# MaxInGaussian/SCFGP

Hardware: AMD Instinct MI355X
Metric: NLML+grad evals/sec (higher is better)
Workload: dtype f32

## Files before the change

### scfgp_amd/csrc/fmap.hip

```cpp
#include "kernels.h"
#include "tile_engine.h"

#include <algorithm>

#define SMEM_DECL extern __shared__ __attribute__((aligned(16))) char smem_raw[]
#ifndef SCFGP_FMAP_WGM
#define SCFGP_FMAP_WGM 4
#endif
#ifndef SCFGP_FMAP_MIN_WGS
#define SCFGP_FMAP_MIN_WGS 6144
#endif
#ifndef SCFGP_FMAP_REG
#define SCFGP_FMAP_REG 1
#endif
#ifndef SCFGP_FMAP_REG_MIN_WGS
#define SCFGP_FMAP_REG_MIN_WGS 16384
#endif
typedef TileCfg<double, 128, 64, 16, SCFGP_FMAP_WGM, 2, 16, true> FmapCfg;

template <typename T>
__global__ __launch_bounds__(FmapCfg::THREADS) void featuremap_kernel(
    const double* __restrict__ Xt, const double* __restrict__ Fall, const Scal* __restrict__ sc,
    T* __restrict__ Phi, int Dp, int Jp, int Kp, int J, int64_t N, int njt, int ncs) {
    typedef FmapCfg Cfg;
    SMEM_DECL;
    double* smem = reinterpret_cast<double*>(smem_raw);
    const int cs = blockIdx.x % ncs;
    const int64_t rb = blockIdx.x / ncs;
    const int per = (njt + ncs - 1) / ncs, jt0 = cs * per, nseg = (jt0 + per <= njt ? per : njt - jt0);
    if (nseg <= 0) return;
    const int nkt = Dp / Cfg::BK;
    TrLoader<double, double, Cfg::BM, Cfg::BK, Cfg::LDA, Cfg::THREADS, false, Cfg::SWZA> la(Xt + rb * Cfg::BM * Dp, Dp, threadIdx.x);
    NatLoader<double, double, Cfg::BN, Cfg::BK, Cfg::LDB, Cfg::THREADS, false, false> lb(Fall + jt0 * Cfg::BN, Jp, threadIdx.x);
    typename Cfg::MTr::acc_t acc[Cfg::TM][Cfg::TN];
    acc_zero<Cfg>(acc);
    const double s = sc->s;
    const T s_hi = (T)s, s_lo = (T)(s - (double)s_hi);
    AccCoord<Cfg> co;
    tile_mainloop_segments<Cfg>(la, lb, nkt, nseg, -(int64_t)Dp, (int64_t)Cfg::BN - (int64_t)Dp * Jp, acc, smem,
        [&](int seg, typename Cfg::MTr::acc_t (&a)[Cfg::TM][Cfg::TN]) {
            T vs[Cfg::TM][Cfg::TN][Cfg::MTr::NACC], vc[Cfg::TM][Cfg::TN][Cfg::MTr::NACC];
#pragma unroll
            for (int tm = 0; tm < Cfg::TM; ++tm)
#pragma unroll
                for (int tn = 0; tn < Cfg::TN; ++tn)
#pragma unroll
                    for (int r = 0; r < Cfg::MTr::NACC; ++r) {
                        T sn, cs_;
                        fast_sincos(a[tm][tn][r], sn, cs_);
                        vc[tm][tn][r] = fma(cs_, s_hi, cs_ * s_lo);
                        vs[tm][tn][r] = fma(sn, s_hi, sn * s_lo);
                    }
#pragma unroll
            for (int tm = 0; tm < Cfg::TM; ++tm)
#pragma unroll
                for (int r = 0; r < Cfg::MTr::NACC; ++r) {
                    const int64_t n = rb * Cfg::BM + co.row(tm, r);
                    T* __restrict__ prow = Phi + n * Kp;
#pragma unroll
                    for (int tn = 0; tn < Cfg::TN; ++tn) {
                        const int j = (jt0 + seg) * Cfg::BN + co.col(tn);
                        if (j < J) {
                            prow[j] = n < N ? vc[tm][tn][r] : (T)0;
                            prow[J + j] = n < N ? vs[tm][tn][r] : (T)0;
                        }
                    }
                }
        });
}

template <typename T, int NK>
__global__ __launch_bounds__(256) void featuremap_reg_kernel(
    const double* __restrict__ A, int lda, const double* __restrict__ Fall, const Scal* __restrict__ sc,
    T* __restrict__ Phi, int Jp, int Kp, int J, int64_t N, int nct, int ncs) {
    typedef MT<double, 16> M;
    typedef T tv2 __attribute__((ext_vector_type(2)));
    const int lane = threadIdx.x & 63, wave = threadIdx.x >> 6, q = lane >> 4, i = lane & 15;
    const int cs = blockIdx.x % ncs;
    const int64_t rb = blockIdx.x / ncs;
    const int per = (nct + ncs - 1) / ncs, ct0 = cs * per, nseg = ct0 + per <= nct ? per : nct - ct0;
    if (nseg <= 0) return;
    const int64_t row0 = rb * 128 + wave * 32;
    double a[2][NK];
#pragma unroll
    for (int tm = 0; tm < 2; ++tm)
#pragma unroll
        for (int ks = 0; ks < NK; ++ks) a[tm][ks] = A[(row0 + tm * 16 + i) * lda + ks * 4 + q];
    const double* bp = Fall + (int64_t)q * Jp + ct0 * 32 + 2 * i;
    v2d b[NK];
#pragma unroll
    for (int ks = 0; ks < NK; ++ks) b[ks] = *reinterpret_cast<const v2d*>(bp + (int64_t)ks * 4 * Jp);
    const double s = sc->s;
    const T s_hi = (T)s, s_lo = (T)(s - (double)s_hi);
    const bool vec = (J & 1) == 0;
    for (int seg = 0; seg < nseg; ++seg) {
        v4d acc[2][2];
#pragma unroll
        for (int tm = 0; tm < 2; ++tm)
#pragma unroll
            for (int tn = 0; tn < 2; ++tn) acc[tm][tn] = v4d{0, 0, 0, 0};
#pragma unroll
        for (int ks = 0; ks < NK; ++ks)
#pragma unroll
            for (int tm = 0; tm < 2; ++tm)
#pragma unroll
                for (int tn = 0; tn < 2; ++tn) M::mfma(acc[tm][tn], a[tm][ks], b[ks][tn]);
        bp += 32;
        if (seg + 1 < nseg) {
#pragma unroll
            for (int ks = 0; ks < NK; ++ks) b[ks] = *reinterpret_cast<const v2d*>(bp + (int64_t)ks * 4 * Jp);
        }
        const int c = (ct0 + seg) * 32 + 2 * i;
        T vs[2][4][2], vc[2][4][2];
#pragma unroll
        for (int tm = 0; tm < 2; ++tm)
#pragma unroll
            for (int r = 0; r < 4; ++r)
#pragma unroll
                for (int tn = 0; tn < 2; ++tn) {
                    T sn, cs_;
                    fast_sincos(acc[tm][tn][r], sn, cs_);
                    vc[tm][r][tn] = fma(cs_, s_hi, cs_ * s_lo);
                    vs[tm][r][tn] = fma(sn, s_hi, sn * s_lo);
                }
#pragma unroll
        for (int tm = 0; tm < 2; ++tm)
#pragma unroll
            for (int r = 0; r < 4; ++r) {
                const int64_t n = row0 + tm * 16 + M::crow(lane, r);
                T* __restrict__ prow = Phi + n * Kp;
                const bool live = n < N;
                const T c0 = live ? vc[tm][r][0] : (T)0, c1 = live ? vc[tm][r][1] : (T)0;
                const T s0 = live ? vs[tm][r][0] : (T)0, s1 = live ? vs[tm][r][1] : (T)0;
                if (vec) {
                    if (c < J) {
                        *reinterpret_cast<tv2*>(prow + c) = tv2{c0, c1};
                        *reinterpret_cast<tv2*>(prow + J + c) = tv2{s0, s1};
                    }
                } else {
                    if (c < J) { prow[c] = c0; prow[J + c] = s0; }
                    if (c + 1 < J) { prow[c + 1] = c1; prow[J + c + 1] = s1; }
                }
            }
    }
}

__global__ __launch_bounds__(FmapCfg::THREADS) void project_kernel(
    const double* __restrict__ Xt, const double* __restrict__ Lall, double* __restrict__ Tt, int Dp, int Sp, int Spp, int njt) {
    typedef FmapCfg Cfg;
    SMEM_DECL;
    double* smem = reinterpret_cast<double*>(smem_raw);
    const int jt = blockIdx.x % njt;
    const int64_t rb = blockIdx.x / njt;
    TrLoader<double, double, Cfg::BM, Cfg::BK, Cfg::LDA, Cfg::THREADS, false, Cfg::SWZA> la(Xt + rb * Cfg::BM * Dp, Dp, threadIdx.x);
    NatLoader<double, double, Cfg::BN, Cfg::BK, Cfg::LDB, Cfg::THREADS, false, false> lb(Lall + jt * Cfg::BN, Spp, threadIdx.x);
    typename Cfg::MTr::acc_t acc[Cfg::TM][Cfg::TN];
    acc_zero<Cfg>(acc);
    tile_mainloop<Cfg>(la, lb, Dp / Cfg::BK, acc, smem);
    AccCoord<Cfg> co;
#pragma unroll
    for (int tm = 0; tm < Cfg::TM; ++tm)
#pragma unroll
        for (int tn = 0; tn < Cfg::TN; ++tn) {
            const int j = jt * Cfg::BN + co.col(tn);
            if (j >= Sp) continue;
#pragma unroll
            for (int r = 0; r < Cfg::MTr::NACC; ++r) Tt[(rb * Cfg::BM + co.row(tm, r)) * Sp + j] = acc[tm][tn][r];
        }
}

template <typename T>
void FmapKernels<T>::featuremap(const Geom& g, const double* Xt, const Projection& pr, const Scal* sc, T* Phi, hipStream_t st) {
    const int njt = g.Jp / FmapCfg::BN;
    const int64_t nrb = g.Np / FmapCfg::BM;
    int ncs = (int)std::min<int64_t>(njt, std::max<int64_t>(1, (SCFGP_FMAP_MIN_WGS + nrb - 1) / nrb));
    const auto launch = [&](auto kernel, const double* A, const double* Bm, int Kd) {
        allow_big_lds(kernel, FmapCfg::LDS_BYTES);
        hipLaunchKernelGGL(kernel, dim3((unsigned)(ncs * nrb)), dim3(FmapCfg::THREADS), FmapCfg::LDS_BYTES, st,
                           A, Bm, sc, Phi, Kd, g.Jp, g.Kp, g.J, g.N, njt, ncs);
    };
    const double *A = Xt, *Bm = pr.Fall; int Kd = g.Dp;
    if (g.lowrank) {
        const int Spp = (int)round_up(g.Sp, FmapCfg::BN), njs = Spp / FmapCfg::BN;
        allow_big_lds(project_kernel, FmapCfg::LDS_BYTES);
        hipLaunchKernelGGL(project_kernel, dim3((unsigned)(njs * nrb)), dim3(FmapCfg::THREADS), FmapCfg::LDS_BYTES, st,
                           Xt, pr.Lall, pr.Tt, g.Dp, g.Sp, Spp, njs);
        A = pr.Tt; Bm = pr.Rall; Kd = g.Sp;
    }
    const int live = (g.lowrank ? g.S : g.D) + 1, nk = (live + 3) / 4;
    if (SCFGP_FMAP_REG && nk <= 9) {
        const int nct = g.Jp / 32;
        const int rcs = (int)std::min<int64_t>(nct, std::max<int64_t>(1, (SCFGP_FMAP_REG_MIN_WGS + nrb - 1) / nrb));
        const auto reg = [&](auto kernel) {
            hipLaunchKernelGGL(kernel, dim3((unsigned)(rcs * nrb)), dim3(256), 0, st, A, Kd, Bm, sc, Phi, g.Jp, g.Kp, g.J, g.N, nct, rcs);
        };
        if (nk <= 3 && Kd >= 12) { reg(featuremap_reg_kernel<T, 3>); return; }
        if (nk <= 4 && Kd >= 16) { reg(featuremap_reg_kernel<T, 4>); return; }
        if (nk <= 5 && Kd >= 20) { reg(featuremap_reg_kernel<T, 5>); return; }
        if (nk <= 8 && Kd >= 32) { reg(featuremap_reg_kernel<T, 8>); return; }
        if (Kd >= 36) { reg(featuremap_reg_kernel<T, 9>); return; }
    }
    launch(featuremap_kernel<T>, A, Bm, Kd);
}

template <typename T>
__global__ void convert_kernel(const double* __restrict__ src, T* __restrict__ dst, int K, int Kp) {
    const int64_t n = (int64_t)Kp * Kp;
    for (int64_t i = (int64_t)blockIdx.x * blockDim.x + threadIdx.x; i < n; i += (int64_t)gridDim.x * blockDim.x) {
        const int r = (int)(i / Kp), c = (int)(i % Kp);
        dst[i] = (r < K && c < K) ? (T)src[i] : (T)0;
    }
}
template <typename T>
__global__ void convert_t_kernel(const double* __restrict__ src, T* __restrict__ dst, int K, int Kp) {
    const int64_t n = (int64_t)Kp * Kp;
    for (int64_t i = (int64_t)blockIdx.x * blockDim.x + threadIdx.x; i < n; i += (int64_t)gridDim.x * blockDim.x) {
        const int k = (int)(i / Kp), j = (int)(i % Kp);
        dst[i] = (k < K && j < K) ? (T)src[(int64_t)j * Kp + k] : (T)0;
    }
}
template <typename T>
void FmapKernels<T>::convert_transposed(const double* src, T* dst, int K, int Kp, hipStream_t st) {
    hipLaunchKernelGGL(convert_t_kernel<T>, dim3(2048), dim3(256), 0, st, src, dst, K, Kp);
}
template <typename T>
void FmapKernels<T>::convert(const double* src, T* dst, int K, int Kp, hipStream_t st) {
    hipLaunchKernelGGL(convert_kernel<T>, dim3(2048), dim3(256), 0, st, src, dst, K, Kp);
}
template struct FmapKernels<double>;
template struct FmapKernels<float>;
__device__ __forceinline__ double scale_x(double x, int mode, const double* __restrict__ sp, int D, int d) {
    if (mode == 0) return x;
    const double mn = sp[d], mx = sp[D + d], lm = sp[2 * D + d], mu = sp[3 * D + d], sd = sp[4 * D + d];
    if (mode == 1) return (x - mn) / (mx - mn);
    if (mode == 2) return (x - mu) / sd;
    if (mode == 3) return 0.5 * erfc(-((x - mu) / sd) * 0.70710678118654752440);
    const double t = (x - mn) / (mx - mn);
    const double bc = ((t < 0 ? -1.0 : (t > 0 ? 1.0 : 0.0)) * pow(fabs(t), lm) - 1.0) / lm;
    const double z = (bc - mu) / sd;
    return mode == 4 ? z : 0.5 * erfc(-z * 0.70710678118654752440);
}
__device__ __forceinline__ double scale_x_deriv(double x, int mode, const double* __restrict__ sp, int D, int d) {
    if (mode == 0) return 1.0;
    const double mn = sp[d], mx = sp[D + d], lm = sp[2 * D + d], mu = sp[3 * D + d], sd = sp[4 * D + d];
    const double inv_sqrt_2pi = 0.39894228040143267794;
// ... 48 lines not shown
```

### scfgp_amd/csrc/kernels.h

```cpp
#pragma once
#include "common.h"

struct Geom {
    int D, S, M, J, K, P;
    int Dp;
    int Jp;
    int Sp;
    int lowrank;
    int Kp;
    int tile;
    int gfull;
    int gstrip;
    int64_t N;
    int64_t Np;
};

struct RowSplits {
    int nsplit;
    int groups;
    int units;
    int taper;
    int gran;
    int64_t nrb;
    __host__ __device__ int per_group() const { return units + taper; }
    __host__ __device__ void range(int s, int64_t& r0, int64_t& r1) const {
        const int pg = per_group(), grp = s / pg, i = s % pg;
        const int64_t g0 = nrb * grp / groups, g1 = nrb * (grp + 1) / groups, len = g1 - g0;
        const int64_t den = (int64_t)1 << taper;
        const int k = i - (units - 1);
        int64_t e0, e1;
        if (taper == 0 || k < 0) { e0 = den * i; e1 = e0 + den; }
        else {
            const int64_t base = den * (units - 1);
            e0 = base + den - (den >> k);
            e1 = k == taper ? base + den : base + den - (den >> (k + 1));
        }
        r0 = (g0 + len * e0 / (den * units)) * gran;
        r1 = (g0 + len * e1 / (den * units)) * gran;
    }
};
RowSplits gram_row_splits(int jobs_per_split, int64_t Np, bool f32, int nsplit_override, int taper);

struct Projection { const double* Fall; const double* Lall; const double* Rall; double* Tt; };

template <typename T>
struct FmapKernels {
    static void featuremap(const Geom& g, const double* Xt, const Projection& pr, const Scal* sc, T* Phi, hipStream_t st);
    static void convert(const double* src, T* dst, int K, int Kp, hipStream_t st);
    static void convert_transposed(const double* src, T* dst, int K, int Kp, hipStream_t st);
};

template <typename T>
struct GramKernels {
    static void gram(const Geom& g, const T* Phi, const double* w, const double* side, const RowSplits& rs, int64_t chunk,
                     double* slabs, double* sidepart, int* qhead, float* ws2, hipStream_t st);
    static int gram_jobs(const Geom& g);
    static void xtz(const Geom& g, const double* Xt, const T* Phi, const T* Phibar, int nsplit, int64_t chunk, double* slabs,
                    hipStream_t st);
    static void zbar_inplace(const Geom& g, const T* Phi, T* Phibar, hipStream_t st);
    static void rsel(const Geom& g, const double* params, T* out, hipStream_t st);
    static void tn_plain(const double* A, int Dp, const T* Bm, int64_t ldb, int J, int64_t Np, int nsplit, int64_t chunk, double* slabs,
                         hipStream_t st);
};

struct F16Operands { const unsigned* Phi16; const char* B16; const float* scale; unsigned* V16; const float* vbound; };

template <typename T>
struct ApplyKernels {
    static void apply_v(const Geom& g, const T* Phi, const T* Bm, T* V, double* vpart, const double* alpha, double* mupart,
                        hipStream_t st, int dma = 0, const F16Operands* f16 = nullptr);
    static void apply_predict(const Geom& g, const T* Phi, const T* LiT, double* vpart, const double* alpha, double* mupart,
                              hipStream_t st);
    static void apply_c(const Geom& g, const T* Phi, const T* LiT, const T* Li, T* C, double* vpart, const double* alpha,
                        const double* beta, double* mupart, hipStream_t st, int dma = 0);
    static void apply_vc(const Geom& g, const T* C, const T* Li, const T* LiT, T* V, hipStream_t st, int dma = 0);
    static void apply_phibar(const Geom& g, const T* Phi, const T* Abar, T* V, const double* p, const double* q,
                             const double* y, const double* alpha, const double* ut, hipStream_t st, int dma = 0, const F16Operands* f16 = nullptr);
    static void apply_plain(const Geom& g, const T* A, const T* Bm, T* Out, int Kc, int ncols, hipStream_t st);
    static void rowstats(const Geom& g, const double* mupart, const double* vpart, const double* y,
                         const Scal* sc, double* p, double* q, double* partial, int nblocks, hipStream_t st);
    static void rowpredict(const Geom& g, const double* mupart, const double* vpart, const Scal* sc, double* mu, double* sd,
                           hipStream_t st);
    static void rowresidual(const Geom& g, const double* mupart, const double* y, double* r, hipStream_t st);
};

struct F16x3Kernels {
    static void split_operand(const Geom& g, const double* M, char* B16, float* scale, double* part, const Scal* sc, hipStream_t st);
    template <int EPI, int BN>
    static int apply(const Geom& g, int njt, int col0, int slot0, const float* Phi, const F16Operands& f, float* V,
                     double* vpart, const double* p, const double* q, const double* y, const double* alpha, const double* ut, double* mu,
                     hipStream_t st, int64_t rb0, int64_t nrb);
    static bool apply_runs(const Geom& g);
    static constexpr size_t F16_PAD = 1024;
    static int side_blocks(const Geom& g);
    static void split_phi(const Geom& g, const float* Phi, const double* y, const Scal* sc, unsigned* Phi16, double* sidepart, float* tmp,
                          hipStream_t st);
// ... 126 lines not shown
```

### scfgp_amd/csrc/scfgp_api.hip

```cpp
#include "../../include/scfgp_hip.h"
#include "kernels.h"

#include <dlfcn.h>
#if __has_include(<rccl/rccl.h>)
#include <rccl/rccl.h>
#else
extern "C" {
typedef struct ncclComm* ncclComm_t;
typedef struct { char internal[128]; } ncclUniqueId;
typedef enum { ncclSuccess = 0 } ncclResult_t;
typedef enum { ncclFloat64 = 8 } ncclDataType_t;
typedef enum { ncclSum = 0 } ncclRedOp_t;
ncclResult_t ncclGetUniqueId(ncclUniqueId*);
ncclResult_t ncclCommInitRank(ncclComm_t*, int, ncclUniqueId, int);
ncclResult_t ncclAllReduce(const void*, void*, size_t, ncclDataType_t, ncclRedOp_t, ncclComm_t, hipStream_t);
ncclResult_t ncclCommDestroy(ncclComm_t);
const char* ncclGetErrorString(ncclResult_t);
}
#endif

#include <algorithm>
#include <cmath>
#include <cstdlib>
#include <cstring>
// ... 20 lines not shown
#ifndef SCFGP_ERR_PER_COND
#define SCFGP_ERR_PER_COND 3.0e-7
#endif
static void derive_geom(Geom& g, int D, int S, int M);

thread_local bool g_scfgp_capturing = false;

struct Roctx {
    int (*push)(const char*) = nullptr; int (*pop)() = nullptr;
    Roctx() {
        void* h = dlopen("librocprofiler-sdk-roctx.so", RTLD_LAZY | RTLD_LOCAL);
        if (!h) h = dlopen("libroctx64.so", RTLD_LAZY | RTLD_LOCAL);
        if (!h) return;
        push = (int (*)(const char*))dlsym(h, "roctxRangePushA");
        pop = (int (*)())dlsym(h, "roctxRangePop");
        if (!push || !pop) { push = nullptr; pop = nullptr; }
    }
};
static Roctx& roctx() { static Roctx r; return r; }

struct Rccl {
    void* h = nullptr;
    decltype(&ncclGetUniqueId) get_id = nullptr; decltype(&ncclCommInitRank) init_rank = nullptr;
    decltype(&ncclAllReduce) all_reduce = nullptr; decltype(&ncclCommDestroy) destroy = nullptr;
    decltype(&ncclGetErrorString) err_string = nullptr;
    bool resolved = false;
    bool bind(void* from) {
        get_id = (decltype(get_id))dlsym(from, "ncclGetUniqueId"); init_rank = (decltype(init_rank))dlsym(from, "ncclCommInitRank");
        all_reduce = (decltype(all_reduce))dlsym(from, "ncclAllReduce"); destroy = (decltype(destroy))dlsym(from, "ncclCommDestroy");
        err_string = (decltype(err_string))dlsym(from, "ncclGetErrorString");
        return get_id && init_rank && all_reduce && destroy && err_string;
    }
    Rccl() {
        if (dlsym(RTLD_DEFAULT, "ncclAllReduce") && bind(RTLD_DEFAULT)) { resolved = true; return; }
        const char* names[] = {"librccl.so", "librccl.so.1", "/opt/rocm/lib/librccl.so.1"};
        for (const char* n : names) if (!h) h = dlopen(n, RTLD_NOW | RTLD_NOLOAD | RTLD_LOCAL);
        for (const char* n : names) if (!h) h = dlopen(n, RTLD_NOW | RTLD_LOCAL);
        if (!h) return;
        if (bind(h)) resolved = true;
        else { dlclose(h); h = nullptr; }
    }
    bool ok() const { return resolved; }
};
static Rccl& rccl() { static Rccl r; return r; }

struct ProfRec { std::string name; hipEvent_t e0, e1; };

struct scfgp_ctx {
    Geom g{};
    int dtype = 0, device = 0;
    hipStream_t st = nullptr; bool own_stream = false;
    hipStream_t copy_st = nullptr; hipEvent_t ev_factor = nullptr;
    int lowrank_bwd = -1; int Spp = 0, Sq = 0; bool last_lrb = false;
    bool want_lrb() const {
        const bool fits = g.lowrank && g.Jp + (int)round_up(g.S, 64) <= g.Kp;
        return fits && (lowrank_bwd == 1 || (lowrank_bwd < 0 && g.Dp >= 4 * g.Sp));
    }
    double* x3_scalars() { return d_x3 + (int64_t)Dpp * g.Jp; }
    double* xs1() { return d_xp1 + n_pk + g.Kp; }
    double* xs2() { return d_xp2 + n_pk + g.Kp; }
    bool unsettled = false; int test_deny_level = 0, test_fail_stage = 0;
    int cap() const { return esc_denied > 0 ? esc_denied - 1 : 2; }
    double* x3_xu() { return d_x3 + (int64_t)Dpp * g.Jp + 8; }
    hipEvent_t ev_fence = nullptr;
    ncclComm_t comm = nullptr; int comm_ranks = 0, comm_rank = 0;
    double* h_pin = nullptr;
    int64_t Ncap = 0, Nglobal = 0, Nglobal_full = 0;
    bool have_params = false, have_data = false;
    int stage = 0, last_want_grad = 0;
    std::vector<double> h_params;
    double *d_params = nullptr, *d_F = nullptr, *d_Fall = nullptr, *d_Lall = nullptr, *d_Rall = nullptr; Scal* d_sc = nullptr;
    double *d_Tt = nullptr, *p_Tt = nullptr;
    double *d_Xraw = nullptr, *d_yraw = nullptr; int64_t Nstore = 0, store_cap = 0; bool work_full = false;
    int64_t* d_idx = nullptr; int64_t idx_cap = 0;
    double *d_Xt = nullptr, *d_y = nullptr, *d_p = nullptr, *d_q = nullptr, *d_mu = nullptr, *d_vpart = nullptr;
    void *d_Phi = nullptr, *d_V = nullptr;
    bool split16 = false; unsigned* d_Phi16 = nullptr; char* d_B16 = nullptr; float* d_f16scale = nullptr;
    unsigned* d_V16g = nullptr; unsigned* d_qV16g = nullptr; double* d_f16side = nullptr; float* d_f16tmp = nullptr;
    int f16gram = 1;
    bool f16_on() const { return split16 && dma() == 2; }
    int64_t f16_chunk() const {
        const int64_t top = gram_chunk > 0 ? 2 * gram_chunk : 8192, fill = g.Np * F16x3Kernels::gram_tiles(g) / 512 / 512 * 512;
        return std::max<int64_t>(std::min(top, fill), 1024);
    }
    bool f16_gram() const { return f16_on() && f16gram && !last_cform; }
    F16Operands f16ops() const { return F16Operands{d_Phi16, d_B16, d_f16scale, nullptr, d_f16tmp + 5}; }
    double *d_xp1 = nullptr, *d_xp2 = nullptr; int64_t n_xp = 0, n_pk = 0;
    double *d_x1 = nullptr, *d_x2 = nullptr, *d_x3 = nullptr; int64_t n_x1 = 0, n_x2 = 0, n_x3 = 0; int Dpp = 0;
    double *d_Li = nullptr, *d_B = nullptr, *d_T1 = nullptr, *d_T2 = nullptr, *d_Abar = nullptr;
    void *d_BT = nullptr, *d_AbarT = nullptr;
    int apply_dma = -1;
    double *d_vecs = nullptr;
    double *d_scalars = nullptr, *d_yy = nullptr; int* d_flag = nullptr;
    float* d_ws2 = nullptr;
    double *d_slabs = nullptr; size_t slabs_bytes = 0;
    double *d_partial = nullptr; int64_t n_partial = 0;
    double *d_work = nullptr, *d_grad = nullptr;
    int xs_mode = 0; double* d_xscale = nullptr;
    int ys_mode = 0; double* d_yscale = nullptr;
    double *p_Xt = nullptr, *p_vpart = nullptr, *p_mupart = nullptr; void *p_Phi = nullptr;
    void *p_FT = nullptr, *p_C = nullptr, *p_V = nullptr, *p_Li = nullptr;
    double *u_Li = nullptr, *u_S = nullptr, *u_Lm = nullptr, *u_Mi = nullptr, *u_Si = nullptr, *u_vec = nullptr, *u_acc = nullptr, *u_part = nullptr;
    double *u_y = nullptr, *u_r = nullptr, *u_slabs = nullptr; size_t u_slabs_bytes = 0;
    void* u_LiT = nullptr; float* u_ws2 = nullptr; int* u_flag = nullptr;
    double *l_y = nullptr, *l_r = nullptr, *l_rec = nullptr, *l_out = nullptr, *l_acc = nullptr; unsigned long long* l_bad = nullptr;
    int opt_algo = -1; OptHyper opt_h{}; double *d_opt = nullptr, *d_tctr = nullptr, *d_hist = nullptr; int hist_cap = 0;
// ... 287 lines not shown
        dfree(c->d_Xraw); dfree(c->d_yraw); c->store_cap = 0;
        if (int rc = dmalloc(c, &c->d_Xraw, sizeof(double) * N * c->g.D)) return rc;
        if (int rc = dmalloc(c, &c->d_yraw, sizeof(double) * N)) return rc;
        c->store_cap = N;
    }
    c->Nstore = N; c->Nglobal_full = n_global > 0 ? n_global : N;
    HIPCHK(c, hipMemcpyAsync(c->d_Xraw, X, sizeof(double) * N * c->g.D, hipMemcpyHostToDevice, c->st));
    HIPCHK(c, hipMemcpyAsync(c->d_yraw, y, sizeof(double) * N, hipMemcpyHostToDevice, c->st));
    if (int rc = load_working_set(c, nullptr, N, n_global)) return rc;
    HIPCHK(c, hipStreamSynchronize(c->st));
    return SCFGP_OK;
}

static void unpack_exchange(scfgp_ctx* c, const double* xp, double* x) {
    const Geom& g = c->g;
    unpack_tri_tiles(xp, g.Kp / g.tile, g.tile, x, g.Kp, c->st);
    hipMemcpyAsync(x + (int64_t)g.Kp * g.Kp, xp + c->n_pk, sizeof(double) * (g.Kp + 8), hipMemcpyDeviceToDevice, c->st);
}

template <typename T> struct Impl {
    typedef SweepKernels<T> SK;
    static void gram_to(scfgp_ctx* c, const T* Mx, const double* w, const double* side, double* out, const char* name) {
        const Geom& g = c->g;
        const int nts = g.Kp / g.tile, ntiles = nts * (nts + 1) / 2;
        if constexpr (sizeof(T) == 4) {
            if (c->f16_gram()) {
                const int nch = F16x3Kernels::gram_chunks(g, c->f16_chunk());
                { ProfScope ps(c, w ? "split_v" : "split_phi");
                  if (w) F16x3Kernels::split_v(g, (const float*)Mx, w, side, F16x3Kernels::apply_runs(g) ? nullptr : c->d_V16g, c->d_qV16g,
                                               c->d_f16side, c->d_f16tmp, c->st);
                  else F16x3Kernels::split_phi(g, (const float*)Mx, side, c->d_sc, c->d_Phi16, c->d_f16side, c->d_f16tmp, c->st); }
                { ProfScope ps(c, name);
                  F16x3Kernels::gram(g, w ? c->d_V16g : c->d_Phi16, w ? c->d_qV16g : c->d_Phi16, c->d_f16tmp + 4, c->f16_chunk(), c->d_slabs, c->st); }
                { ProfScope ps(c, "reduce_tiles"); reduce_tri_tiles(c->d_slabs, nch, nts, g.tile, out, c->st);
                  reduce_side(c->d_f16side, F16x3Kernels::side_blocks(g), g.Kp, g.gfull * g.tile + g.gstrip * 64, out + c->n_pk, c->st); }
                return;
            }
        }
        const int gs = c->splits.nsplit;
        double* sidepart = c->d_slabs + (size_t)gs * ntiles * g.tile * g.tile;
        { ProfScope ps(c, name);
          SK::gram(g, Mx, w, side, c->splits, c->dtype == SCFGP_F32 ? c->gram_chunk : 0, c->d_slabs, sidepart, c->d_flag + 8, c->d_ws2, c->st); }
        { ProfScope ps(c, "reduce_tiles"); reduce_tri_tiles(c->d_slabs, gs, nts, g.tile, out, c->st);
          reduce_side(sidepart, gs, g.Kp, g.gfull * g.tile + g.gstrip * 64, out + c->n_pk, c->st); }
    }
    static int pass1(scfgp_ctx* c) {
        const Geom& g = c->g;
        if (!c->in_train) HIPCHK(c, hipMemsetAsync(c->d_flag, 0, sizeof(int) * 4, c->st));
        const bool use64 = sizeof(T) == 4 && c->use64();
        c->last_cform = c->want_cform();
        if ((use64 && c->phi64_cap < g.Np) || (c->last_cform && c->c_cap < g.Np)) {
            c->err = "pass1: auxiliary row buffer missing"; return SCFGP_EARG;
        }
        const Projection proj{c->d_Fall, c->d_Lall, c->d_Rall, c->d_Tt};
        if constexpr (sizeof(T) == 4) {
            if (use64) {
                typedef SweepKernels<double> SK64;
                const int nts = g.Kp / g.tile, ntiles = nts * (nts + 1) / 2, gs = c->splits64.nsplit;
                double* sidepart = c->d_slabs + (size_t)gs * ntiles * g.tile * g.tile;
                { ProfScope ps(c, "featuremap64"); SK64::featuremap(g, c->d_Xt, proj, c->d_sc, (double*)c->d_Phi64, c->st); }
                { ProfScope ps(c, "gram64");
                  SK64::gram(g, (const double*)c->d_Phi64, nullptr, c->d_y, c->splits64, 0, c->d_slabs, sidepart, c->d_flag + 8, nullptr, c->st); }
                { ProfScope ps(c, "reduce_tiles"); reduce_tri_tiles(c->d_slabs, gs, nts, g.tile, c->d_xp1, c->st);
                  reduce_side(sidepart, gs, g.Kp, g.gfull * g.tile + g.gstrip * 64, c->d_xp1 + c->n_pk, c->st); }
            }
        }
        { ProfScope ps(c, "featuremap"); SK::featuremap(g, c->d_Xt, proj, c->d_sc, (T*)c->d_Phi, c->st); }
        if constexpr (sizeof(T) == 4) {
            if (c->f16_on() && (use64 || !c->f16_gram())) {
                ProfScope ps(c, "split_phi");
                F16x3Kernels::split_phi(g, (const float*)c->d_Phi, c->d_y, c->d_sc, c->d_Phi16, c->d_f16side, c->d_f16tmp, c->st);
            }
        }
        if (!use64) gram_to(c, (const T*)c->d_Phi, nullptr, c->d_y, c->d_xp1, "gram");
        c->last_used64 = use64 || sizeof(T) == 8; c->last_level = sizeof(T) == 8 ? 0 : c->level();
        HIPCHK(c, hipMemcpyAsync(c->xs1(), c->d_yy, sizeof(double), hipMemcpyDeviceToDevice, c->st));
        write_status(c->xs1(), c->last_level >= 1 ? 1.0 : 0.0, c->cap() < 1 ? 1.0 : 0.0, c->cap() < 2 ? 1.0 : 0.0, 0.0, c->st);
        HIPCHK(c, hipGetLastError());
        return SCFGP_OK;
    }
    static int factor(scfgp_ctx* c) {
        const Geom& g = c->g;
        { ProfScope ps(c, "kstage_factor");
          hipMemcpyAsync(c->d_x1 + (int64_t)g.Kp * g.Kp, c->d_xp1 + c->n_pk, sizeof(double) * (g.Kp + 8), hipMemcpyDeviceToDevice, c->st);
          kstage_factor(c->kstage(), c->d_xp1, c->d_sc, c->st); }
        if (c->last_cform) {
            SK::convert(c->d_Li, (T*)c->d_BT, g.K, g.Kp, c->st);
            SK::convert_transposed(c->d_Li, (T*)c->d_AbarT, g.K, g.Kp, c->st);
        } else {
            SK::convert(c->d_B, (T*)c->d_BT, g.K, g.Kp, c->st);
            if (c->f16_on()) {
                F16x3Kernels::split_operand(g, c->d_B, c->d_B16, c->d_f16scale, c->d_partial, c->d_sc, c->st);
                F16x3Kernels::v_bound(g, c->d_B, c->d_sc, c->d_f16tmp, c->st);
            }
        }
        HIPCHK(c, hipGetLastError());
        return SCFGP_OK;
    }
    static int pass2(scfgp_ctx* c, int want_grad) {
        const Geom& g = c->g;
        if (c->last_cform) {
            const int dma = c->dma() ? 1 : 0;
            { ProfScope ps(c, "apply_c");
              SK::apply_c(g, (const T*)c->d_Phi, (const T*)c->d_AbarT, (const T*)c->d_BT, (T*)c->d_C, c->d_vpart, c->alpha(), c->beta(), c->d_mu, c->st, dma); }
            { ProfScope ps(c, "apply_vc");
              SK::apply_vc(g, (const T*)c->d_C, (const T*)c->d_BT, (const T*)c->d_AbarT, (T*)c->d_V, c->st, dma); }
        } else {
// ... 1554 lines not shown

extern "C" int scfgp_get_timings(scfgp_ctx* c, double* ms, const char** names, int n) {
    if (!c) return SCFGP_EARG;
    hipStreamSynchronize(c->st);
    int k = 0;
    for (const ProfRec& r : c->recs) {
        if (k >= n) break;
        float t = 0;
        if (hipEventElapsedTime(&t, r.e0, r.e1) != hipSuccess) t = -1;
        if (ms) ms[k] = t;
        if (names) names[k] = r.name.c_str();
        ++k;
    }
    return k;
}

static void derive_geom(Geom& g, int D, int S, int M) {
    g.D = D; g.S = S; g.M = M; g.J = S + M; g.K = 2 * g.J; g.P = 3 + D * S + M * S + S + M;
    g.Dp = (int)round_up(D + 1, 16); g.Jp = (int)round_up(g.J, XT);
    g.Sp = (int)round_up(S + 1, 16); g.lowrank = g.Sp < g.Dp;
    g.tile = 128;
    g.gfull = (int)(round_up(g.K, 64) / 128);
    g.gstrip = (int)(round_up(g.K, 64) / 64 % 2);
    g.Kp = (g.gfull + g.gstrip) * g.tile;
}
extern "C" int scfgp_selftest_row_splits(int D, int S, int M, int64_t N, int dtype, int nsplit, int taper) {
    if (D < 1 || S < 1 || M < 1 || N < 1) return SCFGP_EARG;
    Geom g{};
    derive_geom(g, D, S, M);
    g.N = N; g.Np = round_up(N, 256);
    const int jobs = dtype == SCFGP_F32 ? SweepKernels<float>::gram_jobs(g) : SweepKernels<double>::gram_jobs(g);
    const RowSplits rs = gram_row_splits(jobs, g.Np, dtype == SCFGP_F32, nsplit, taper);
    if (rs.nsplit < 1 || rs.nsplit != rs.groups * rs.per_group()) return 1;
    int64_t at = 0;
    for (int s = 0; s < rs.nsplit; ++s) {
        int64_t r0, r1; rs.range(s, r0, r1);
        if (r0 != at || r1 < r0 || r0 % rs.gran || r1 % rs.gran || (rs.gran != 64 && rs.gran != 256)) return 2;
        at = r1;
    }
    return at == g.Np ? 0 : 3;
}

extern "C" int scfgp_set_option(scfgp_ctx* c, const char* name, int64_t value) {
    if (!c || !name) return SCFGP_EARG;
    const std::string s(name);
    if (s == "gram_nsplit") c->gram_nsplit = (int)value;
    else if (s == "gram_taper") c->gram_taper = (int)value;
    else if (s == "apply_dma") { if (value < -1 || value > 2) { c->err = "apply_dma: -1 auto, 0 off, 1 = 128-wide tiles, 2 = 256-wide (fp32)"; return SCFGP_EARG; }
                                 c->apply_dma = (int)value; }
    else if (s == "gram_chunk") c->gram_chunk = value;
    else if (s == "f16_gram") c->f16gram = (int)value;
    else if (s == "lowrank_bwd") c->lowrank_bwd = (int)value;
    else if (s == "xtz_nsplit") c->xtz_nsplit = (int)value;
    else if (s == "use_graph") c->use_graph = (int)value;
    else if (s == "gram64") { if (value < 0 || value > 3) { c->err = "gram64: 0 never, 1 always level 1, 2 auto, 3 always level 2"; return SCFGP_EARG; }
                              c->gram64 = (int)value; c->esc_level = 0; c->esc_denied = 0; }
    else if (s == "factor_form") { if (value < -1 || value > 1) { c->err = "factor_form: -1 auto, 0 never, 1 always"; return SCFGP_EARG; } c->factor_form = (int)value; }
    else if (s == "cond_threshold") c->esc_thr = (double)value;
    else if (s == "cond_threshold_w") c->escw_thr = (double)value;
    else if (s == "roctx") c->roctx_on = value != 0;
    else if (s == "test_deny_level") { c->test_deny_level = (int)value; return SCFGP_OK; }
    else if (s == "test_fail_stage") { c->test_fail_stage = (int)value; return SCFGP_OK; }
    else { c->err = "unknown option " + s; return SCFGP_EARG; }
    c->warm = false; c->cond_valid = false;
    if (c->gexec) { hipGraphExecDestroy(c->gexec); c->gexec = nullptr; }
    if (c->graph) { hipGraphDestroy(c->graph); c->graph = nullptr; }
    if (c->have_data) return ensure_rows(c, c->g.N);
    return SCFGP_OK;
}

extern "C" int scfgp_get_condition(scfgp_ctx* c, double* out, int n) {
    if (!c || !out || n < 4) return SCFGP_EARG;
    const double v[9] = {c->cond_est(), (double)c->last_level, c->last_used64 ? 1.0 : 0.0, c->alpha_err_fp32(),
                         c->esc_thr, c->escw_thr, c->cond[0], c->cond[1], c->cond[2]};
    for (int i = 0; i < n && i < 9; ++i) out[i] = v[i];
    return SCFGP_OK;
}

extern "C" int64_t scfgp_debug_read(scfgp_ctx* c, const char* name, void* host, int64_t max_bytes) {
    if (!c || !name || !host) return SCFGP_EARG;
    const Geom& g = c->g;
    const std::string s(name);
    if (s == "chol_trace") { if (hipStreamSynchronize(c->st) != hipSuccess) return SCFGP_EHIP; return chol_trace_read(host, max_bytes); }
    if (s == "apply_trace") { if (hipStreamSynchronize(c->st) != hipSuccess) return SCFGP_EHIP; return apply_trace_read(host, max_bytes); }
    if (s == "trace") { if (hipStreamSynchronize(c->st) != hipSuccess) return SCFGP_EHIP; return trace_read(host, max_bytes); }
    const int64_t K2 = (int64_t)g.Kp * g.Kp;
    const size_t ts = c->tsize();
    const void* src = nullptr; int64_t bytes = 0;
    DevTmp tmp;
    if (s == "Phi") { src = c->d_Phi; bytes = ts * g.Np * g.Kp; }
    else if (s == "V") { src = c->d_V; bytes = ts * g.Np * g.Kp; }
    else if (s == "G") {
        if (dmalloc(c, &tmp.p, 8 * c->n_x1)) return SCFGP_EHIP;
        unpack_exchange(c, c->d_xp1, tmp.p); src = tmp.p; bytes = 8 * c->n_x1;
    }
    else if (s == "W") { if (c->stage == 3) unpack_exchange(c, c->d_xp2, c->d_x2); src = c->d_x2; bytes = 8 * c->n_x2; }
    else if (s == "XZ") { src = c->d_x3; bytes = 8 * c->n_x3; }
    else if (s == "Li") { src = c->d_Li; bytes = 8 * K2; }
    else if (s == "B") { src = c->d_B; bytes = 8 * K2; }
    else if (s == "Abar") { src = c->d_Abar; bytes = 8 * K2; }
    else if (s == "p") { src = c->d_p; bytes = 8 * g.Np; }
    else if (s == "q") { src = c->d_q; bytes = 8 * g.Np; }
    else if (s == "vecs") { src = c->d_vecs; bytes = 8 * 5 * g.Kp; }
    else if (s == "Fall") { src = c->d_Fall; bytes = 8 * (int64_t)g.Dp * g.Jp; }
    else if (s == "Lall") { src = c->d_Lall; bytes = 8 * (int64_t)g.Dp * round_up(g.Sp, 64); }
    else if (s == "Rall") { src = c->d_Rall; bytes = 8 * (int64_t)g.Sp * g.Jp; }
// ... 32 lines not shown
```

### scfgp_amd/csrc/sincos.h

```cpp
#pragma once
#include "common.h"

__device__ __forceinline__ void fast_sincos(double z, double& sn, double& cs) {
    const double fn = rint(z * 6.36619772367581382433e-01);
    const double r = fma(-fn, 1.57079632673412561417e+00, z);
    const double w = fn * 6.07710050650619224932e-11;
    const double x = r - w;
    const double y = (r - x) - w;
    const double z2 = x * x;
    const double S1 = -1.66666666666666324348e-01, S2 = 8.33333333332248946124e-03, S3 = -1.98412698298579493134e-04,
                 S4 = 2.75573137070700676789e-06, S5 = -2.50507602534068634195e-08, S6 = 1.58969099521155010221e-10;
    const double v = z2 * x;
    const double rs = S2 + z2 * (S3 + z2 * (S4 + z2 * (S5 + z2 * S6)));
    const double s = x - ((z2 * (0.5 * y - v * rs) - y) - v * S1);
    const double C1 = 4.16666666666666019037e-02, C2 = -1.38888888888741095749e-03, C3 = 2.48015872894767294178e-05,
                 C4 = -2.75573143513906633035e-07, C5 = 2.08757232129817482790e-09, C6 = -1.13596475577881948265e-11;
    const double rc = z2 * (C1 + z2 * (C2 + z2 * (C3 + z2 * (C4 + z2 * (C5 + z2 * C6)))));
    const double hz = 0.5 * z2;
    const double wc = 1.0 - hz;
    const double c = wc + (((1.0 - wc) - hz) + (z2 * rc - x * y));
    const int q = (int)fn & 3;
    const double ss = (q & 1) ? c : s, cc = (q & 1) ? s : c;
    sn = (q & 2) ? -ss : ss;
    cs = ((q + 1) & 2) ? -cc : cc;
}

__device__ __forceinline__ void fast_sincos(double z, float& sn, float& cs) {
    const double fn = rint(z * 6.36619772367581382433e-01);
    const double r = fma(-fn, 6.07710050650619224932e-11, fma(-fn, 1.57079632673412561417e+00, z));
    const float x = (float)r, z2 = x * x;
    const float s = fmaf(x * z2, fmaf(z2, fmaf(z2, -1.9515295891e-4f, 8.3321608736e-3f), -1.6666654611e-1f), x);
    const float c = fmaf(z2 * z2, fmaf(z2, fmaf(z2, 2.443315711809948e-5f, -1.388731625493765e-3f), 4.166664568298827e-2f),
                         fmaf(-0.5f, z2, 1.0f));
    const int q = (int)fn & 3;
    const float ss = (q & 1) ? c : s, cc = (q & 1) ? s : c;
    sn = (q & 2) ? -ss : ss;
    cs = ((q + 1) & 2) ? -cc : cc;
}
```

Baseline: 4.986.

## Software-pipeline feature-map MFMA with packed sincos epilogue and occupancy hints

The register-resident feature-map kernel now double-buffers accumulators. It computes the next column segment's MFMAs while the current segment's sincos and stores run, and interleaves them with sched_group_barrier hints. The f32 sincos is evaluated two lanes at a time with packed float FMAs. Launch bounds now request a minimum occupancy, and an ncs override option is added. The aim is to hide MFMA latency behind the transcendental epilogue, at the cost of more registers and code complexity.

```diff
diff --git a/scfgp_amd/csrc/fmap.hip b/scfgp_amd/csrc/fmap.hip
--- a/scfgp_amd/csrc/fmap.hip
+++ b/scfgp_amd/csrc/fmap.hip
@@ -39,17 +39,21 @@
     AccCoord<Cfg> co;
     tile_mainloop_segments<Cfg>(la, lb, nkt, nseg, -(int64_t)Dp, (int64_t)Cfg::BN - (int64_t)Dp * Jp, acc, smem,
         [&](int seg, typename Cfg::MTr::acc_t (&a)[Cfg::TM][Cfg::TN]) {
+            typedef T tv2 __attribute__((ext_vector_type(2)));
+            const tv2 sh = tv2{s_hi, s_hi}, sl = tv2{s_lo, s_lo};
             T vs[Cfg::TM][Cfg::TN][Cfg::MTr::NACC], vc[Cfg::TM][Cfg::TN][Cfg::MTr::NACC];
+            static_assert(Cfg::MTr::NACC % 2 == 0, "the phases of a lane go through sin / cos two by two");
 #pragma unroll
             for (int tm = 0; tm < Cfg::TM; ++tm)
 #pragma unroll
                 for (int tn = 0; tn < Cfg::TN; ++tn)
 #pragma unroll
-                    for (int r = 0; r < Cfg::MTr::NACC; ++r) {
-                        T sn, cs_;
-                        fast_sincos(a[tm][tn][r], sn, cs_);
-                        vc[tm][tn][r] = fma(cs_, s_hi, cs_ * s_lo);
-                        vs[tm][tn][r] = fma(sn, s_hi, sn * s_lo);
+                    for (int r = 0; r < Cfg::MTr::NACC; r += 2) {
+                        tv2 sn, cn;
+                        fast_sincos2(a[tm][tn][r], a[tm][tn][r + 1], sn, cn);
+                        const tv2 c2 = fma2(cn, sh, cn * sl), s2 = fma2(sn, sh, sn * sl);
+                        vc[tm][tn][r] = c2[0]; vc[tm][tn][r + 1] = c2[1];
+                        vs[tm][tn][r] = s2[0]; vs[tm][tn][r + 1] = s2[1];
                     }
 #pragma unroll
             for (int tm = 0; tm < Cfg::TM; ++tm)
@@ -69,12 +73,17 @@
         });
 }
 
+template <int NK>
+__device__ __forceinline__ void fmap_reg_mfma(v4d (&acc)[2][2], const double (&a)[2][NK], const v2d (&b)[NK], int m) {
+    MT<double, 16>::mfma(acc[(m >> 1) & 1][m & 1], a[(m >> 1) & 1][m >> 2], b[m >> 2][m & 1]);
+}
 template <typename T, int NK>
-__global__ __launch_bounds__(256) void featuremap_reg_kernel(
+__global__ __launch_bounds__(256, NK <= 4 ? 3 : 2) void featuremap_reg_kernel(
     const double* __restrict__ A, int lda, const double* __restrict__ Fall, const Scal* __restrict__ sc,
     T* __restrict__ Phi, int Jp, int Kp, int J, int64_t N, int nct, int ncs) {
     typedef MT<double, 16> M;
     typedef T tv2 __attribute__((ext_vector_type(2)));
+    constexpr int VPM = (sizeof(T) == 4 ? 448 : 896) / (4 * NK);
     const int lane = threadIdx.x & 63, wave = threadIdx.x >> 6, q = lane >> 4, i = lane & 15;
     const int cs = blockIdx.x % ncs;
     const int64_t rb = blockIdx.x / ncs;
@@ -92,56 +101,96 @@
     for (int ks = 0; ks < NK; ++ks) b[ks] = *reinterpret_cast<const v2d*>(bp + (int64_t)ks * 4 * Jp);
     const double s = sc->s;
     const T s_hi = (T)s, s_lo = (T)(s - (double)s_hi);
+    const tv2 sh = tv2{s_hi, s_hi}, sl = tv2{s_lo, s_lo};
     const bool vec = (J & 1) == 0;
-    for (int seg = 0; seg < nseg; ++seg) {
-        v4d acc[2][2];
-#pragma unroll
-        for (int tm = 0; tm < 2; ++tm)
-#pragma unroll
-            for (int tn = 0; tn < 2; ++tn) acc[tm][tn] = v4d{0, 0, 0, 0};
-#pragma unroll
-        for (int ks = 0; ks < NK; ++ks)
+    v4d acc0[2][2], acc1[2][2];
+#pragma unroll
+    for (int tm = 0; tm < 2; ++tm)
+#pragma unroll
+        for (int tn = 0; tn < 2; ++tn) acc0[tm][tn] = v4d{0, 0, 0, 0};
+#pragma unroll
+    for (int m = 0; m < 4 * NK; ++m) fmap_reg_mfma<NK>(acc0, a, b, m);
+    if (nseg > 1) {
+        bp += 32;
+#pragma unroll
+        for (int ks = 0; ks < NK; ++ks) b[ks] = *reinterpret_cast<const v2d*>(bp + (int64_t)ks * 4 * Jp);
+    }
+    const auto step = [&](v4d (&acc)[2][2], v4d (&nxt)[2][2], int seg) __attribute__((always_inline)) {
+        const int c = (ct0 + seg) * 32 + 2 * i;
+        const bool more = seg + 1 < nseg;
+        const double* bn = bp + (seg + 2 < nseg ? 32 : 0);
+        if (more && vec && (ct0 + seg) * 32 + 32 <= J) {
 #pragma unroll
             for (int tm = 0; tm < 2; ++tm)
 #pragma unroll
-                for (int tn = 0; tn < 2; ++tn) M::mfma(acc[tm][tn], a[tm][ks], b[ks][tn]);
-        bp += 32;
-        if (seg + 1 < nseg) {
-#pragma unroll
-            for (int ks = 0; ks < NK; ++ks) b[ks] = *reinterpret_cast<const v2d*>(bp + (int64_t)ks * 4 * Jp);
-        }
-        const int c = (ct0 + seg) * 32 + 2 * i;
-        T vs[2][4][2], vc[2][4][2];
-#pragma unroll
-        for (int tm = 0; tm < 2; ++tm)
-#pragma unroll
-            for (int r = 0; r < 4; ++r)
-#pragma unroll
-                for (int tn = 0; tn < 2; ++tn) {
-                    T sn, cs_;
-                    fast_sincos(acc[tm][tn][r], sn, cs_);
-                    vc[tm][r][tn] = fma(cs_, s_hi, cs_ * s_lo);
-                    vs[tm][r][tn] = fma(sn, s_hi, sn * s_lo);
+                for (int tn = 0; tn < 2; ++tn) nxt[tm][tn] = v4d{0, 0, 0, 0};
+#pragma unroll
+            for (int g = 0; g < 8; ++g) {
+#pragma unroll
+                for (int m = g * 4 * NK / 8; m < (g + 1) * 4 * NK / 8; ++m) {
+                    fmap_reg_mfma<NK>(nxt, a, b, m);
+                    if ((m & 3) == 3) b[m >> 2] = *reinterpret_cast<const v2d*>(bn + (int64_t)(m >> 2) * 4 * Jp);
                 }
-#pragma unroll
-        for (int tm = 0; tm < 2; ++tm)
-#pragma unroll
-            for (int r = 0; r < 4; ++r) {
+                const int tm = g >> 2, r = g & 3;
+                tv2 sn, cn;
+                fast_sincos2(acc[tm][0][r], acc[tm][1][r], sn, cn);
+                const tv2 vc = fma2(cn, sh, cn * sl), vs = fma2(sn, sh, sn * sl);
                 const int64_t n = row0 + tm * 16 + M::crow(lane, r);
                 T* __restrict__ prow = Phi + n * Kp;
                 const bool live = n < N;
-                const T c0 = live ? vc[tm][r][0] : (T)0, c1 = live ? vc[tm][r][1] : (T)0;
-                const T s0 = live ? vs[tm][r][0] : (T)0, s1 = live ? vs[tm][r][1] : (T)0;
-                if (vec) {
-                    if (c < J) {
-                        *reinterpret_cast<tv2*>(prow + c) = tv2{c0, c1};
-                        *reinterpret_cast<tv2*>(prow + J + c) = tv2{s0, s1};
+                *reinterpret_cast<tv2*>(prow + c) = live ? vc : tv2{0, 0};
+                *reinterpret_cast<tv2*>(prow + J + c) = live ? vs : tv2{0, 0};
+            }
+#pragma unroll
+            for (int m = 0; m < 4 * NK; ++m) {
+                __builtin_amdgcn_sched_group_barrier(0x008, 1, 0);
+                __builtin_amdgcn_sched_group_barrier(0x002, VPM, 0);
+            }
+        } else {
+            if (more) {
+#pragma unroll
+                for (int tm = 0; tm < 2; ++tm)
+#pragma unroll
+                    for (int tn = 0; tn < 2; ++tn) nxt[tm][tn] = v4d{0, 0, 0, 0};
+#pragma unroll
+                for (int m = 0; m < 4 * NK; ++m) fmap_reg_mfma<NK>(nxt, a, b, m);
+#pragma unroll
+                for (int ks = 0; ks < NK; ++ks) b[ks] = *reinterpret_cast<const v2d*>(bn + (int64_t)ks * 4 * Jp);
+            }
+            tv2 vs[2][4], vc[2][4];
+#pragma unroll
+            for (int tm = 0; tm < 2; ++tm)
+#pragma unroll
+                for (int r = 0; r < 4; ++r) {
+                    tv2 sn, cn;
+                    fast_sincos2(acc[tm][0][r], acc[tm][1][r], sn, cn);
+                    vc[tm][r] = fma2(cn, sh, cn * sl);
+                    vs[tm][r] = fma2(sn, sh, sn * sl);
+                }
+#pragma unroll
+            for (int tm = 0; tm < 2; ++tm)
+#pragma unroll
+                for (int r = 0; r < 4; ++r) {
+                    const int64_t n = row0 + tm * 16 + M::crow(lane, r);
+                    T* __restrict__ prow = Phi + n * Kp;
+                    const bool live = n < N;
+                    const tv2 cv = live ? vc[tm][r] : tv2{0, 0}, sv = live ? vs[tm][r] : tv2{0, 0};
+                    if (vec) {
+                        if (c < J) {
+                            *reinterpret_cast<tv2*>(prow + c) = cv;
+                            *reinterpret_cast<tv2*>(prow + J + c) = sv;
+                        }
+                    } else {
+                        if (c < J) { prow[c] = cv[0]; prow[J + c] = sv[0]; }
+                        if (c + 1 < J) { prow[c + 1] = cv[1]; prow[J + c + 1] = sv[1]; }
                     }
-                } else {
-                    if (c < J) { prow[c] = c0; prow[J + c] = s0; }
-                    if (c + 1 < J) { prow[c + 1] = c1; prow[J + c + 1] = s1; }
                 }
-            }
+        }
+        bp = bn;
+    };
+    for (int seg = 0; seg < nseg; seg += 2) {
+        step(acc0, acc1, seg);
+        if (seg + 1 < nseg) step(acc1, acc0, seg + 1);
     }
 }
 
@@ -174,6 +223,7 @@
     const int njt = g.Jp / FmapCfg::BN;
     const int64_t nrb = g.Np / FmapCfg::BM;
     int ncs = (int)std::min<int64_t>(njt, std::max<int64_t>(1, (SCFGP_FMAP_MIN_WGS + nrb - 1) / nrb));
+    if (pr.ncs > 0) ncs = std::min(njt, pr.ncs);
     const auto launch = [&](auto kernel, const double* A, const double* Bm, int Kd) {
         allow_big_lds(kernel, FmapCfg::LDS_BYTES);
         hipLaunchKernelGGL(kernel, dim3((unsigned)(ncs * nrb)), dim3(FmapCfg::THREADS), FmapCfg::LDS_BYTES, st,
@@ -190,7 +240,8 @@
     const int live = (g.lowrank ? g.S : g.D) + 1, nk = (live + 3) / 4;
     if (SCFGP_FMAP_REG && nk <= 9) {
         const int nct = g.Jp / 32;
-        const int rcs = (int)std::min<int64_t>(nct, std::max<int64_t>(1, (SCFGP_FMAP_REG_MIN_WGS + nrb - 1) / nrb));
+        int rcs = (int)std::min<int64_t>(nct, std::max<int64_t>(1, (SCFGP_FMAP_REG_MIN_WGS + nrb - 1) / nrb));
+        if (pr.ncs > 0) rcs = std::min(nct, pr.ncs);
         const auto reg = [&](auto kernel) {
             hipLaunchKernelGGL(kernel, dim3((unsigned)(rcs * nrb)), dim3(256), 0, st, A, Kd, Bm, sc, Phi, g.Jp, g.Kp, g.J, g.N, nct, rcs);
         };
diff --git a/scfgp_amd/csrc/kernels.h b/scfgp_amd/csrc/kernels.h
--- a/scfgp_amd/csrc/kernels.h
+++ b/scfgp_amd/csrc/kernels.h
@@ -41,7 +41,7 @@
 };
 RowSplits gram_row_splits(int jobs_per_split, int64_t Np, bool f32, int nsplit_override, int taper);
 
-struct Projection { const double* Fall; const double* Lall; const double* Rall; double* Tt; };
+struct Projection { const double* Fall; const double* Lall; const double* Rall; double* Tt; int ncs = 0; };
 
 template <typename T>
 struct FmapKernels {
diff --git a/scfgp_amd/csrc/scfgp_api.hip b/scfgp_amd/csrc/scfgp_api.hip
--- a/scfgp_amd/csrc/scfgp_api.hip
+++ b/scfgp_amd/csrc/scfgp_api.hip
@@ -96,6 +96,7 @@
     hipStream_t st = nullptr; bool own_stream = false;
     hipStream_t copy_st = nullptr; hipEvent_t ev_factor = nullptr;
     int lowrank_bwd = -1; int Spp = 0, Sq = 0; bool last_lrb = false;
+    int fmap_ncs = 0;
     bool want_lrb() const {
         const bool fits = g.lowrank && g.Jp + (int)round_up(g.S, 64) <= g.Kp;
         return fits && (lowrank_bwd == 1 || (lowrank_bwd < 0 && g.Dp >= 4 * g.Sp));
@@ -489,7 +490,7 @@
         if ((use64 && c->phi64_cap < g.Np) || (c->last_cform && c->c_cap < g.Np)) {
             c->err = "pass1: auxiliary row buffer missing"; return SCFGP_EARG;
         }
-        const Projection proj{c->d_Fall, c->d_Lall, c->d_Rall, c->d_Tt};
+        const Projection proj{c->d_Fall, c->d_Lall, c->d_Rall, c->d_Tt, c->fmap_ncs};
         if constexpr (sizeof(T) == 4) {
             if (use64) {
                 typedef SweepKernels<double> SK64;
@@ -2150,6 +2151,7 @@
     else if (s == "f16_gram") c->f16gram = (int)value;
     else if (s == "lowrank_bwd") c->lowrank_bwd = (int)value;
     else if (s == "xtz_nsplit") c->xtz_nsplit = (int)value;
+    else if (s == "fmap_ncs") { if (value < 0) { c->err = "fmap_ncs: 0 = by the launch's rule, n > 0 = n column ranges per row block"; return SCFGP_EARG; } c->fmap_ncs = (int)value; }
     else if (s == "use_graph") c->use_graph = (int)value;
     else if (s == "gram64") { if (value < 0 || value > 3) { c->err = "gram64: 0 never, 1 always level 1, 2 auto, 3 always level 2"; return SCFGP_EARG; }
                               c->gram64 = (int)value; c->esc_level = 0; c->esc_denied = 0; }
diff --git a/scfgp_amd/csrc/sincos.h b/scfgp_amd/csrc/sincos.h
--- a/scfgp_amd/csrc/sincos.h
+++ b/scfgp_amd/csrc/sincos.h
@@ -37,3 +37,30 @@
     sn = (q & 2) ? -ss : ss;
     cs = ((q + 1) & 2) ? -cc : cc;
 }
+
+typedef float v2f __attribute__((ext_vector_type(2)));
+__device__ __forceinline__ v2f fma2(v2f a, v2f b, v2f c) { return __builtin_elementwise_fma(a, b, c); }
+__device__ __forceinline__ v2d fma2(v2d a, v2d b, v2d c) { return __builtin_elementwise_fma(a, b, c); }
+__device__ __forceinline__ void fast_sincos2(double z0, double z1, v2d& sn, v2d& cs) {
+    double s0, c0, s1, c1;
+    fast_sincos(z0, s0, c0);
+    fast_sincos(z1, s1, c1);
+    sn = v2d{s0, s1};
+    cs = v2d{c0, c1};
+}
+__device__ __forceinline__ void fast_sincos2(double z0, double z1, v2f& sn, v2f& cs) {
+    const double fn0 = rint(z0 * 6.36619772367581382433e-01), fn1 = rint(z1 * 6.36619772367581382433e-01);
+    const double r0 = fma(-fn0, 6.07710050650619224932e-11, fma(-fn0, 1.57079632673412561417e+00, z0));
+    const double r1 = fma(-fn1, 6.07710050650619224932e-11, fma(-fn1, 1.57079632673412561417e+00, z1));
+    const v2f x = v2f{(float)r0, (float)r1}, z2 = x * x;
+    const v2f S1 = -1.6666654611e-1f, S2 = 8.3321608736e-3f, S3 = -1.9515295891e-4f;
+    const v2f C1 = 4.166664568298827e-2f, C2 = -1.388731625493765e-3f, C3 = 2.443315711809948e-5f;
+    const v2f half = -0.5f, one = 1.0f;
+    const v2f s = fma2(x * z2, fma2(z2, fma2(z2, S3, S2), S1), x);
+    const v2f c = fma2(z2 * z2, fma2(z2, fma2(z2, C3, C2), C1), fma2(half, z2, one));
+    const int q0 = (int)fn0 & 3, q1 = (int)fn1 & 3;
+    const float ss0 = (q0 & 1) ? c[0] : s[0], cc0 = (q0 & 1) ? s[0] : c[0];
+    const float ss1 = (q1 & 1) ? c[1] : s[1], cc1 = (q1 & 1) ? s[1] : c[1];
+    sn = v2f{(q0 & 2) ? -ss0 : ss0, (q1 & 2) ? -ss1 : ss1};
+    cs = v2f{((q0 + 1) & 2) ? -cc0 : cc0, ((q1 + 1) & 2) ? -cc1 : cc1};
+}
```

Result: no change. 5.000, median of 6 (+0.3%).
